# surrealdb/surrealdb

Hardware: AMD Instinct MI355X
Metric: knn_qps (higher is better)
Workload: dtype f32; 1 GPU; brute-force cosine KNN, 10000000 rows/GPU x 768-dim f32, K=10, single query (BASELINE configs[1]); batch=0, rows_total=10000000, rows_per_gpu=10000000, dim=768, k=10, distance=cosine, parallelism=single

## Files before the change

surrealdb_amd/csrc/sdbv.hip:

```cpp

#include <hip/hip_runtime.h>
#include <rocblas/rocblas.h>

#include <algorithm>
#include <atomic>
#include <cfloat>
#include <chrono>
#include <cmath>
#include <cstdint>
#include <deque>
#include <limits>
#include <memory>
#include <thread>
#include <unordered_set>
#include <cstdio>
#include <cstring>
#include <map>
#include <mutex>
#include <queue>
#include <set>
#include <string>
#include <unordered_map>
#include <vector>

// ... 360 lines not shown
	sum.f = __fadd_rn(sum.f, __fadd_rn(p[0].f, p[4].f));                        \
	sum.f = __fadd_rn(sum.f, __fadd_rn(p[1].f, p[5].f));                        \
	sum.f = __fadd_rn(sum.f, __fadd_rn(p[2].f, p[6].f));                        \
	sum.f = __fadd_rn(sum.f, __fadd_rn(p[3].f, p[7].f));
				COMB(x) COMB(y) COMB(z) COMB(w)
#undef COMB
				for (; k8 < d; k8++) {
					const float4 v =
					    *(const float4 *)(cm + (uint64_t)k8 * n_pad + r0);
					const float qk = qs[k8];
					sum.x = __fadd_rn(sum.x, __fmul_rn(v.x, qk));
					sum.y = __fadd_rn(sum.y, __fmul_rn(v.y, qk));
					sum.z = __fadd_rn(sum.z, __fmul_rn(v.z, qk));
					sum.w = __fadd_rn(sum.w, __fmul_rn(v.w, qk));
				}
				const float s[4] = {sum.x, sum.y, sum.z, sum.w};
#pragma unroll
				for (int c = 0; c < ROWS_PER_LANE; c++) {
					double den = q_norm * norms[r0 + c < n_pad ? r0 + c : 0];
					dist[c] = 1.0 - (double)s[c] / den;
				}
			} else {
				float4 acc = make_float4(0.f, 0.f, 0.f, 0.f);
				for (uint32_t kk = 0; kk < d; kk++) {
					const float4 v =
					    *(const float4 *)(cm + (uint64_t)kk * n_pad + r0);
					const float qk = qs[kk];
					float dx = v.x - qk, dy = v.y - qk, dz = v.z - qk,
					      dw = v.w - qk;
					acc.x = __fadd_rn(acc.x, __fmul_rn(dx, dx));
					acc.y = __fadd_rn(acc.y, __fmul_rn(dy, dy));
					acc.z = __fadd_rn(acc.z, __fmul_rn(dz, dz));
					acc.w = __fadd_rn(acc.w, __fmul_rn(dw, dw));
				}
				const float s[4] = {acc.x, acc.y, acc.z, acc.w};
#pragma unroll
				for (int c = 0; c < ROWS_PER_LANE; c++)
					dist[c] = sqrt((double)s[c]);
			}
		}

		uint64_t kk_key = kth_key;
		uint32_t kk_row = kth_row;
		int full = (topk_n >= (int)k);
#pragma unroll
		for (int c = 0; c < ROWS_PER_LANE; c++) {
			if (!valid[c])
				continue;
			uint64_t key = d_total_key(dist[c]);
			uint32_t row32 = (uint32_t)(r0 + c);
			bool take = !full || key < kk_key || (key == kk_key && row32 < kk_row);
			if (take) {
				int idx = atomicAdd(&cnt, 1);
				buf[idx].key = key;
				buf[idx].dist = dist[c];
				buf[idx].row = row32;
			}
		}
		__syncthreads();

		if (cnt > 0) {
			int m = cnt;
			for (int i = threadIdx.x; i < topk_n; i += THREADS)
				buf[m + i] = topk[i];
			int total = m + topk_n;
			__syncthreads();
			int new_n;
			block_select_topk(buf, total, topk, (int)k, &new_n);
			if (threadIdx.x == 0) {
				topk_n = new_n;
				if (new_n >= (int)k) {
					kth_key = topk[k - 1].key;
					kth_row = topk[k - 1].row;
				}
				cnt = 0;
			}
		}
		__syncthreads();
	}

	scan_topk_write(topk, topk_n, k, ids, block_out);
}

__device__ __forceinline__ static void merge_slice(
    Cand *__restrict__ block_out, uint64_t total, uint32_t k,
    uint64_t per_block, Cand *__restrict__ out) {
	__shared__ uint64_t red_key[THREADS / 64];
	__shared__ uint64_t red_id[THREADS / 64];
	__shared__ long red_idx[THREADS / 64];
	const int lane = threadIdx.x & 63;
	const int wave = threadIdx.x >> 6;
	const uint64_t s0 = (uint64_t)blockIdx.x * per_block;
	const uint64_t s1 = s0 + per_block < total ? s0 + per_block : total;
	out += (uint64_t)blockIdx.x * k;
	if (s0 >= total) {
		for (uint32_t i = threadIdx.x; i < k; i += THREADS) {
			out[i].dist = __longlong_as_double(0x7FF0000000000000LL);
			out[i].id = ~0ULL;
		}
		return;
	}
	for (int slot = 0; slot < (int)k; slot++) {
		uint64_t bk = ~0ULL;
		uint64_t bid = ~0ULL;
		long bi = -1;
		for (uint64_t i = s0 + threadIdx.x; i < s1; i += THREADS) {
			uint64_t ck = d_total_key(block_out[i].dist);
			uint64_t cid = block_out[i].id;
			if (ck < bk || (ck == bk && cid < bid)) {
				bk = ck;
				bid = cid;
				bi = (long)i;
			}
		}
		for (int off = 32; off > 0; off >>= 1) {
			uint64_t ok = __shfl_down(bk, off);
			uint64_t oid = __shfl_down(bid, off);
			long oi = __shfl_down(bi, off);
			if (ok < bk || (ok == bk && oid < bid)) {
				bk = ok;
				bid = oid;
				bi = oi;
			}
		}
		if (lane == 0) {
			red_key[wave] = bk;
			red_id[wave] = bid;
			red_idx[wave] = bi;
		}
		__syncthreads();
		if (threadIdx.x == 0) {
			uint64_t bbk = ~0ULL, bbid = ~0ULL;
			long best = -1;
			for (int w = 0; w < THREADS / 64; w++) {
				if (red_idx[w] < 0)
					continue;
				if (red_key[w] < bbk ||
				    (red_key[w] == bbk && red_id[w] < bbid)) {
					bbk = red_key[w];
					bbid = red_id[w];
					best = red_idx[w];
				}
			}
			if (best < 0) {
				out[slot].dist =
				    __longlong_as_double(0x7FF0000000000000LL);
				out[slot].id = ~0ULL;
			} else {
				out[slot] = block_out[best];
				block_out[best].dist =
				    __longlong_as_double(0x7FF0000000000000LL);
				block_out[best].id = ~0ULL;
			}
		}
		__syncthreads();
	}
}

__global__ __launch_bounds__(THREADS) void k_merge(
    Cand *__restrict__ block_out, uint64_t total, uint32_t k,
    uint64_t per_block, Cand *__restrict__ out) {
	merge_slice(block_out, total, k, per_block, out);
}

#define PF_ROWS_PER_LANE 8
#define PF_TILE (THREADS * PF_ROWS_PER_LANE)
#define PF_CAND_CAP 16384u
#define PF_RESCORE_BLOCKS 2048
#define PF_NORM_MIN 0x1p-30
#define PF_NORM_MAX 0x1p30

__host__ __device__ static inline uint32_t pf_bf16_bits(uint32_t u) {
	return (u + 0x7FFFu + ((u >> 16) & 1u)) >> 16;
}

__host__ __device__ static inline float pf_eps(uint32_t d) {
	return 1.01f * (0x1p-8f + 2.0f * (float)(d + 8) * 0x1p-24f) + 0x1p-20f;
}

__device__ static inline uint32_t d_key32(float x) {
	uint32_t b = __float_as_uint(x);
	return (b >> 31) ? ~b : (b | 0x80000000u);
}
__device__ static inline float d_unkey32(uint32_t k) {
	return __uint_as_float((k >> 31) ? (k & 0x7FFFFFFFu) : ~k);
}

__global__ void k_shadow(const float *__restrict__ cm,
                         const double *__restrict__ norms,
                         uint16_t *__restrict__ sh, float *__restrict__ pinv,
                         uint64_t n, uint64_t n_pad, uint64_t sn_pad,
                         uint32_t d) {
	uint64_t r0 = ((uint64_t)blockIdx.x * blockDim.x + threadIdx.x) *
	              PF_ROWS_PER_LANE;
	if (r0 >= sn_pad)
		return;
	const bool in_cm = r0 < n_pad;
	uint32_t bad = 0;
	for (uint32_t k = 0; k < d; k++) {
		float4 a = make_float4(0.f, 0.f, 0.f, 0.f), b = a;
		if (in_cm) {
			a = *(const float4 *)(cm + (uint64_t)k * n_pad + r0);
			b = *(const float4 *)(cm + (uint64_t)k * n_pad + r0 + 4);
		}
		const float v[8] = {a.x, a.y, a.z, a.w, b.x, b.y, b.z, b.w};
		uint32_t h[8];
#pragma unroll
		for (int c = 0; c < 8; c++) {
			uint32_t u = __float_as_uint(v[c]);
			h[c] = pf_bf16_bits(u) & 0xFFFFu;
			if ((u & 0x7F800000u) == 0x7F800000u ||
			    (h[c] & 0x7F80u) == 0x7F80u)
				bad |= 1u << c;
		}
		uint4 o;
		o.x = h[0] | (h[1] << 16);
		o.y = h[2] | (h[3] << 16);
		o.z = h[4] | (h[5] << 16);
		o.w = h[6] | (h[7] << 16);
		*(uint4 *)(sh + (uint64_t)k * sn_pad + r0) = o;
	}
#pragma unroll
	for (int c = 0; c < 8; c++) {
		uint64_t r = r0 + c;
		float inv = __uint_as_float(0x7FC00000u);
		if (r < n && !((bad >> c) & 1u)) {
			double nm = norms[r];
			if (nm >= PF_NORM_MIN && nm <= PF_NORM_MAX)
				inv = (float)(1.0 / nm);
		}
		pinv[r] = inv;
	}
}

__device__ static void pf_block_select(uint64_t *buf, int total,
                                       uint64_t *topk, int k, int *out_n) {
	__shared__ uint64_t red_v[THREADS / 64];
	__shared__ int red_i[THREADS / 64];
	const int lane = threadIdx.x & 63;
	const int wave = threadIdx.x >> 6;
	int out = total < k ? total : k;
	for (int slot = 0; slot < out; slot++) {
		uint64_t bv = ~0ULL;
// ... 880 lines not shown
		}
	} else {
		if (threadIdx.x == 0) {
			float acc = 0.f;
			for (uint32_t kk = 0; kk < d; kk++) {
				float diff = xs[kk] - qs[kk];
				acc = __fadd_rn(acc, __fmul_rn(diff, diff));
			}
			Cand o;
			o.dist = sqrt((double)acc);
			o.id = ids[r];
			*out = o;
		}
	}
}

template <int METRIC>
__device__ __forceinline__ static void rows_exact(
    const float *__restrict__ cm, const double *__restrict__ norms,
    const uint64_t *__restrict__ ids, uint64_t n_pad, uint32_t d,
    const float *__restrict__ qg, double q_norm,
    const uint32_t *__restrict__ rows, uint32_t cnt, Cand *__restrict__ out,
    float *qs, float *xs, float *ps) {
	for (uint32_t i = threadIdx.x; i < d; i += 64)
		qs[i] = qg[i];
	for (uint32_t c = blockIdx.x; c < cnt; c += gridDim.x)
		rows_exact_one<METRIC>(cm, norms, ids, n_pad, d, q_norm, rows[c],
		                       out + c, qs, xs, ps);
}

template <int METRIC>
__global__ __launch_bounds__(64) void k_pf_rescore(
    const float *__restrict__ cm, const double *__restrict__ norms,
    const uint64_t *__restrict__ ids, uint64_t n_pad, uint32_t d,
    const float *__restrict__ qg, double q_norm,
    const uint32_t *__restrict__ cand_cnt,
    const uint32_t *__restrict__ cand_rows, Cand *__restrict__ out) {
	__shared__ float qs[MAX_D];
	__shared__ float xs[MAX_D];
	__shared__ float ps[8];
	const uint32_t cnt = *cand_cnt;
	if (cnt > PF_CAND_CAP || blockIdx.x >= cnt)
		return;
	rows_exact<METRIC>(cm, norms, ids, n_pad, d, qg, q_norm, cand_rows, cnt,
	                   out, qs, xs, ps);
}

template <int METRIC>
__global__ __launch_bounds__(64) void k_rows_exact(
    const float *__restrict__ cm, const double *__restrict__ norms,
    const uint64_t *__restrict__ ids, uint64_t n_pad, uint32_t d,
    const float *__restrict__ qg, double q_norm,
    const uint32_t *__restrict__ rows, uint32_t cnt, Cand *__restrict__ out) {
	__shared__ float qs[MAX_D];
	__shared__ float xs[MAX_D];
	__shared__ float ps[8];
	rows_exact<METRIC>(cm, norms, ids, n_pad, d, qg, q_norm, rows, cnt, out,
	                   qs, xs, ps);
}

__global__ __launch_bounds__(THREADS) void k_pf_final(
    Cand *__restrict__ cands, const uint32_t *__restrict__ cand_cnt,
    uint32_t k, Cand *__restrict__ out) {
	const uint32_t raw = *cand_cnt;
	const uint64_t total = raw > PF_CAND_CAP ? 0 : raw;
	if (threadIdx.x == 0) {
		out[k].dist = 0.0;
		out[k].id = raw;
	}
	merge_slice(cands, total, k, total, out);
}

#define PF4_LIST_CAP 262144u
#define PF4_BLOCK_LIST 8192
#define PF4_PASSES 4
#ifndef PF4_REFINE_LANES
#define PF4_REFINE_LANES 32
#endif

__global__ __launch_bounds__(64) void k_pf4_threshold(
    const float *__restrict__ cm, const double *__restrict__ norms,
    const uint64_t *__restrict__ ids, uint64_t n_pad, uint32_t d,
    const float *__restrict__ qg, double q_norm,
    const Cand *__restrict__ approx_top, Cand *__restrict__ out) {
	__shared__ float qs[MAX_D];
	__shared__ float xs[MAX_D];
	__shared__ float ps[8];
	const uint64_t r = approx_top[blockIdx.x].id;
	if (r == ~0ULL) {
		if (threadIdx.x == 0) {
			Cand o;
			o.dist = __longlong_as_double(0x7FF0000000000000LL);
			o.id = ~0ULL;
			out[blockIdx.x] = o;
		}
		return;
	}
	for (uint32_t i = threadIdx.x; i < d; i += 64)
		qs[i] = qg[i];
	rows_exact_one<0>(cm, norms, ids, n_pad, d, q_norm, (uint32_t)r,
	                  out + blockIdx.x, qs, xs, ps);
}

__device__ __forceinline__ static double pf4_threshold(
    const Cand *__restrict__ thr, uint32_t k, unsigned long long *key) {
	if (threadIdx.x == 0)
		*key = 0;
	__syncthreads();
	if (threadIdx.x < k)
		atomicMax(key, (unsigned long long)d_total_key(thr[threadIdx.x].dist));
	__syncthreads();
	const uint64_t kb = *key;
	return __longlong_as_double(
	    (long long)((kb >> 63) ? (kb & 0x7FFFFFFFFFFFFFFFULL) : ~kb));
}

__global__ __launch_bounds__(THREADS) void k_pf4_compact(
    const float *__restrict__ scores, uint64_t n,
    const Cand *__restrict__ thr, uint32_t k, uint32_t list_cap,
    uint32_t *__restrict__ list_cnt, uint32_t *__restrict__ list_rows) {
	__shared__ uint32_t rows[PF4_BLOCK_LIST];
	__shared__ uint32_t cnt, base;
	__shared__ unsigned long long tkey;
	if (threadIdx.x == 0)
		cnt = 0;
	const double T = pf4_threshold(thr, k, &tkey);
	const uint64_t ngrp = (n + 3) / 4;
	const uint64_t round = (uint64_t)THREADS * PF4_PASSES;
	for (uint64_t g0 = (uint64_t)blockIdx.x * round;;
	     g0 += (uint64_t)gridDim.x * round) {
		const bool last = g0 >= ngrp;
		float4 s[PF4_PASSES];
#pragma unroll
		for (int p = 0; p < PF4_PASSES; p++) {
			const uint64_t g = g0 + (uint64_t)p * THREADS + threadIdx.x;
			if (g < ngrp)
				s[p] = *(const float4 *)(scores + g * 4);
		}
#pragma unroll
		for (int p = 0; p < PF4_PASSES; p++) {
			const uint64_t g = g0 + (uint64_t)p * THREADS + threadIdx.x;
			if (g >= ngrp)
				continue;
			const float v[4] = {s[p].x, s[p].y, s[p].z, s[p].w};
#pragma unroll
			for (int c = 0; c < 4; c++) {
				const uint64_t r = g * 4 + c;
				if (r < n && !((double)v[c] > T))
					rows[atomicAdd(&cnt, 1u)] = (uint32_t)r;
			}
		}
		__syncthreads();
		const uint32_t m = cnt;
		__syncthreads();
		if (m > PF4_BLOCK_LIST - 4 * THREADS * PF4_PASSES || (last && m > 0)) {
			if (threadIdx.x == 0) {
				base = atomicAdd(list_cnt, m);
				cnt = 0;
			}
			__syncthreads();
			for (uint32_t i = threadIdx.x; i < m; i += THREADS)
				if (base + i < list_cap)
					list_rows[base + i] = rows[i];
			__syncthreads();
		}
		if (last)
			break;
	}
}

__global__ __launch_bounds__(THREADS) void k_pf4_refine(
// ... 1946 lines not shown
		return SDBV_ERR_NO_TABLE;
	it->second.order = order;
	return SDBV_OK;
}

static int ensure_query_scratch(sdbv_ctx *ctx, uint32_t d, uint64_t nblocks,
                                uint32_t k) {
	if (ctx->q_cap < d) {
		if (ctx->q_dev)
			(void)hipFree(ctx->q_dev);
		const size_t qb = d * sizeof(float) +
		                  (size_t)((d + 31) / 32) * PF6_QWORDS * sizeof(uint32_t);
		HIP_CHECK(ctx, hipMalloc(&ctx->q_dev, qb));
		if (ctx->q_pin)
			(void)hipHostFree(ctx->q_pin);
		HIP_CHECK(ctx, hipHostMalloc(&ctx->q_pin, qb));
		ctx->q_cap = d;
	}
	uint64_t need = nblocks * k * sizeof(Cand);
	if (ctx->block_out_cap < need) {
		if (ctx->block_out)
			(void)hipFree(ctx->block_out);
		HIP_CHECK(ctx, hipMalloc(&ctx->block_out, need));
		ctx->block_out_cap = need;
	}
	if (!ctx->final_out)
		HIP_CHECK(ctx, hipMalloc(&ctx->final_out, MAX_K * sizeof(Cand)));
	if (!ctx->merge_tmp)
		HIP_CHECK(ctx,
		          hipMalloc(&ctx->merge_tmp, 32 * MAX_K * sizeof(Cand)));
	return SDBV_OK;
}

static int stage_query(sdbv_ctx *ctx, const float *q, uint32_t d,
                       size_t q_bytes) {
	std::memcpy(ctx->q_pin, q, d * sizeof(float));
	HIP_CHECK(ctx, hipMemcpyAsync(ctx->q_dev, ctx->q_pin, q_bytes,
	                              hipMemcpyHostToDevice, ctx->stream));
	return SDBV_OK;
}

static void copy_results(const Cand *host_out, uint32_t m, uint64_t *out_ids,
                         double *out_dists, uint32_t *out_n) {
	*out_n = m;
	for (uint32_t i = 0; i < m; i++) {
		out_ids[i] = host_out[i].id;
		out_dists[i] = host_out[i].dist;
	}
}

static uint64_t scan_grid(uint64_t n, uint64_t *rows_per_block) {
	uint64_t tiles = (n + TILE - 1) / TILE;
	uint64_t nblocks = tiles < 2048 ? tiles : 2048;
	if (nblocks == 0)
		nblocks = 1;
	uint64_t tiles_per_block = (tiles + nblocks - 1) / nblocks;
	*rows_per_block = tiles_per_block * TILE;
	return (n + *rows_per_block - 1) / *rows_per_block;
}

static void launch_scan(sdbv_ctx *ctx, Table &t, uint32_t k, double q_norm,
                        uint64_t nblocks, uint64_t rows_per_block,
                        const uint64_t *mask) {
#define LAUNCH_SCAN(M, MASKED)                                                 \
	hipLaunchKernelGGL((k_scan<M, MASKED>), dim3((uint32_t)nblocks),           \
	                   dim3(THREADS), 0, ctx->stream, t.cm, t.norms, t.n,      \
	                   t.n_pad, t.d, ctx->q_dev, q_norm, k, rows_per_block,    \
	                   (Cand *)ctx->block_out, t.ids_dev, mask)
	const bool cosine = t.metric == SDBV_METRIC_COSINE;
	if (mask) {
		if (cosine)
			LAUNCH_SCAN(0, true);
		else
			LAUNCH_SCAN(1, true);
	} else {
		if (cosine)
			LAUNCH_SCAN(0, false);
		else
			LAUNCH_SCAN(1, false);
	}
#undef LAUNCH_SCAN
}

static void launch_merge_tree(sdbv_ctx *ctx, uint64_t nblocks, uint32_t k) {
	uint64_t total = nblocks * k;
	const uint64_t G = 32;
	if (total > 4096 && nblocks > G) {
		uint64_t per = ((nblocks + G - 1) / G) * k;
		hipLaunchKernelGGL(k_merge, dim3((uint32_t)G), dim3(THREADS), 0,
		                   ctx->stream, (Cand *)ctx->block_out, total, k, per,
		                   (Cand *)ctx->merge_tmp);
		hipLaunchKernelGGL(k_merge, dim3(1), dim3(THREADS), 0, ctx->stream,
		                   (Cand *)ctx->merge_tmp, G * k, k, G * k,
		                   (Cand *)ctx->final_out);
	} else {
		hipLaunchKernelGGL(k_merge, dim3(1), dim3(THREADS), 0, ctx->stream,
		                   (Cand *)ctx->block_out, total, k, total,
		                   (Cand *)ctx->final_out);
	}
}

static void launch_all_dists(sdbv_ctx *ctx, Table &t, const float *q,
                             double *dout) {
	uint64_t nb = (t.n + THREADS - 1) / THREADS;
	double q_norm = t.metric == SDBV_METRIC_COSINE
	                    ? sqrt((double)h_sumsq_f32(q, t.d))
	                    : 0;
	double q_mean = t.metric == SDBV_METRIC_PEARSON ? h_mean_f32(q, t.d) : 0;
#define LAUNCH_AD(M)                                                       \
	hipLaunchKernelGGL(k_all_dists<M>, dim3((uint32_t)nb), dim3(THREADS), \
	                   0, ctx->stream, t.cm, t.norms, t.n, t.n_pad, t.d,  \
	                   ctx->q_dev, q_norm, t.order, q_mean, dout)
	switch (t.metric) {
	case SDBV_METRIC_COSINE: LAUNCH_AD(0); break;
	case SDBV_METRIC_EUCLIDEAN: LAUNCH_AD(1); break;
	case SDBV_METRIC_MANHATTAN: LAUNCH_AD(2); break;
	case SDBV_METRIC_CHEBYSHEV: LAUNCH_AD(3); break;
	case SDBV_METRIC_HAMMING: LAUNCH_AD(4); break;
	case SDBV_METRIC_JACCARD:
		hipLaunchKernelGGL(k_jaccard_dists, dim3((uint32_t)t.n), dim3(256),
		                   0, ctx->stream, t.cm, t.n, t.n_pad, t.d,
		                   ctx->q_dev, dout);
		break;
	case SDBV_METRIC_MINKOWSKI: LAUNCH_AD(6); break;
	case SDBV_METRIC_PEARSON: LAUNCH_AD(7); break;
	}
#undef LAUNCH_AD
}

static int knn_large_k(sdbv_ctx *ctx, Table &t, const float *q, uint32_t d,
                       uint32_t k, const uint64_t *allow, uint64_t *out_ids,
                       double *out_dists, uint32_t *out_n) {
	int rc = ensure_query_scratch(ctx, d, 1, 1);
	if (rc != SDBV_OK)
		return rc;
	rc = stage_query(ctx, q, d, d * sizeof(float));
	if (rc != SDBV_OK)
		return rc;
	double *dout = nullptr;
	HIP_CHECK(ctx, hipMalloc(&dout, t.n * sizeof(double)));
	HIP_CHECK(ctx, hipEventRecord(ctx->ev0, ctx->stream));
	launch_all_dists(ctx, t, q, dout);
	HIP_CHECK(ctx, hipEventRecord(ctx->ev1, ctx->stream));
	std::vector<double> hd(t.n);
	std::vector<uint64_t> hids(t.n);
	if (hipMemcpyAsync(hd.data(), dout, t.n * sizeof(double),
	                   hipMemcpyDeviceToHost, ctx->stream) != hipSuccess ||
	    hipMemcpyAsync(hids.data(), t.ids_dev, t.n * sizeof(uint64_t),
	                   hipMemcpyDeviceToHost, ctx->stream) != hipSuccess ||
	    hipStreamSynchronize(ctx->stream) != hipSuccess ||
	    hipGetLastError() != hipSuccess) {
		(void)hipFree(dout);
		ctx->err = "knn_large_k: device error";
		return SDBV_ERR_HIP;
	}
	(void)hipFree(dout);
	float ms = 0;
	(void)hipEventElapsedTime(&ms, ctx->ev0, ctx->ev1);
	ctx->stats.last_scan_kernel_ms = ms;
	ctx->stats.last_merge_kernel_ms = 0;
	if (!allow)
		ctx->stats.last_rows_scanned = t.n;
	auto tkey = [](double x) {
		uint64_t bits;
		std::memcpy(&bits, &x, 8);
		return (bits >> 63) ? ~bits : (bits | 0x8000000000000000ULL);
	};
	std::priority_queue<std::pair<uint64_t, uint64_t>> heap;
	for (uint64_t r = 0; r < t.n; r++) {
		if (allow && !((allow[r >> 6] >> (r & 63)) & 1ULL))
			continue;
		std::pair<uint64_t, uint64_t> e{tkey(hd[r]), r};
		if (heap.size() < k) {
			heap.push(e);
// ... 301 lines not shown
			nb = 2048;
		if (nb == 0)
			nb = 1;
		hipLaunchKernelGGL(k_pf_compact, dim3((uint32_t)nb), dim3(THREADS), 0,
		                   ctx->stream, ctx->pf_scores, t.n,
		                   (const Cand *)ctx->final_out, k,
		                   kind == 1 ? pf_eps(t.d) : 0.0f, cand_cnt,
		                   ctx->pf_rows);
		if (kind == 5)
			hipLaunchKernelGGL(k_pf_rescore<1>, dim3(PF_RESCORE_BLOCKS),
			                   dim3(64), 0, ctx->stream, t.cm, t.norms,
			                   t.ids_dev, t.n_pad, t.d, ctx->q_dev, q_norm,
			                   cand_cnt, ctx->pf_rows, (Cand *)ctx->pf_cands);
		else
			hipLaunchKernelGGL(k_pf_rescore<0>, dim3(PF_RESCORE_BLOCKS),
			                   dim3(64), 0, ctx->stream, t.cm, t.norms,
			                   t.ids_dev, t.n_pad, t.d, ctx->q_dev, q_norm,
			                   cand_cnt, ctx->pf_rows, (Cand *)ctx->pf_cands);
	}
	HIP_CHECK(ctx, hipEventRecord(ctx->ev3, ctx->stream));
	hipLaunchKernelGGL(k_pf_final, dim3(1), dim3(THREADS), 0, ctx->stream,
	                   (Cand *)ctx->pf_cands, cand_cnt, k, res);
	HIP_CHECK(ctx, hipEventRecord(ctx->ev4, ctx->stream));
	HIP_CHECK(ctx, hipMemcpyAsync(host_out, res, (k + 1) * sizeof(Cand),
	                              hipMemcpyDeviceToHost, ctx->stream));
	HIP_CHECK(ctx, hipStreamSynchronize(ctx->stream));
	HIP_CHECK(ctx, hipGetLastError());
	*ncand = (uint32_t)host_out[k].id;

	float ms_pre = 0, ms_sel = 0, ms_rescore = 0, ms_final = 0;
	(void)hipEventElapsedTime(&ms_pre, ctx->ev0, ctx->ev1);
	(void)hipEventElapsedTime(&ms_sel, ctx->ev1, ctx->ev2);
	(void)hipEventElapsedTime(&ms_rescore, ctx->ev2, ctx->ev3);
	(void)hipEventElapsedTime(&ms_final, ctx->ev3, ctx->ev4);
	ctx->stats.last_scan_kernel_ms = (double)ms_pre + ms_rescore;
	ctx->stats.last_merge_kernel_ms = (double)ms_sel + ms_final;
	if (!mask)
		ctx->stats.last_rows_scanned = t.n;
	return SDBV_OK;
}

static uint32_t pf4_list_max() {
	uint64_t cap = PF4_LIST_CAP;
	const char *e = getenv("SDBV_SCAN_PREFILTER_H4_LIST_MAX");
	if (e && *e) {
		uint64_t v = strtoull(e, nullptr, 10);
		if (v < cap)
			cap = v;
	}
	return (uint32_t)cap;
}

static int knn_prefilter_h4(sdbv_ctx *ctx, Table &t, uint32_t k, double q_norm,
                            const PfQ6 &q6, uint32_t list_cap, Cand *host_out,
                            uint32_t *ncand, uint32_t *nstage1) {
	const Shadow &sh = t.sh;
	int rc = ensure_prefilter_scratch(ctx, sh.sn_pad);
	if (rc != SDBV_OK)
		return rc;
	if (!ctx->pf4_list)
		HIP_CHECK(ctx, hipMalloc(&ctx->pf4_list,
		                         PF4_LIST_CAP * sizeof(uint32_t)));
	if (!ctx->pf4_thr)
		HIP_CHECK(ctx, hipMalloc(&ctx->pf4_thr, MAX_K * sizeof(Cand)));

	uint64_t rows_per_block = 0;
	const uint64_t nblocks =
	    prefilter_grid(ctx, t.n, 4, false, &rows_per_block);
	Cand *res = (Cand *)ctx->pf_res;
	uint32_t *cand_cnt = (uint32_t *)&res[MAX_K + 1];
	const uint32_t ngroups = (t.d + 31) / 32;
	const uint32_t *qd = (const uint32_t *)(ctx->q_dev + t.d);
	const Cand *thr = (const Cand *)ctx->pf4_thr;

	HIP_CHECK(ctx, hipEventRecord(ctx->ev0, ctx->stream));
	hipLaunchKernelGGL((k_prefilter_i6<false, true>), dim3((uint32_t)nblocks),
	                   dim3(THREADS), 0, ctx->stream,
	                   (const uint4 *)sh.plane_h(), (const uint2 *)nullptr,
	                   sh.pscale(), sh.peps4(), sh.xsum_h(), t.n, sh.sn_pad,
	                   ngroups, qd, q6.qscale, q6.qeps, q6.bias4, k,
	                   rows_per_block, ctx->pf_scores, (Cand *)ctx->block_out,
	                   cand_cnt, (const uint64_t *)nullptr);
	HIP_CHECK(ctx, hipEventRecord(ctx->ev1, ctx->stream));
	launch_merge_tree(ctx, nblocks, k);
	HIP_CHECK(ctx, hipEventRecord(ctx->ev2, ctx->stream));
	{
		hipLaunchKernelGGL(k_pf4_threshold, dim3(k), dim3(64), 0, ctx->stream,
		                   t.cm, t.norms, t.ids_dev, t.n_pad, t.d, ctx->q_dev,
		                   q_norm, (const Cand *)ctx->final_out,
		                   (Cand *)ctx->pf4_thr);
		uint64_t ngrp = (t.n + 3) / 4;
		uint64_t nb = (ngrp + THREADS * PF4_PASSES - 1) / (THREADS * PF4_PASSES);
		if (nb > 512)
			nb = 512;
		if (nb == 0)
			nb = 1;
		hipLaunchKernelGGL(k_pf4_compact, dim3((uint32_t)nb), dim3(THREADS), 0,
		                   ctx->stream, ctx->pf_scores, t.n, thr, k, list_cap,
		                   cand_cnt + 1, ctx->pf4_list);
		hipLaunchKernelGGL(k_pf4_refine, dim3(2048), dim3(THREADS), 0,
		                   ctx->stream, (const uint4 *)sh.plane_h(),
		                   (const uint2 *)sh.plane_l(t.d), sh.pscale(),
		                   sh.peps(), sh.xsum(), sh.sn_pad, ngroups, qd,
		                   q6.qscale, q6.qeps, q6.bias, thr, k, list_cap,
		                   cand_cnt + 1, ctx->pf4_list, cand_cnt,
		                   ctx->pf_rows);
		hipLaunchKernelGGL(k_pf_rescore<0>, dim3(PF_RESCORE_BLOCKS), dim3(64),
		                   0, ctx->stream, t.cm, t.norms, t.ids_dev, t.n_pad,
		                   t.d, ctx->q_dev, q_norm, cand_cnt, ctx->pf_rows,
		                   (Cand *)ctx->pf_cands);
	}
	HIP_CHECK(ctx, hipEventRecord(ctx->ev3, ctx->stream));
	hipLaunchKernelGGL(k_pf_final, dim3(1), dim3(THREADS), 0, ctx->stream,
	                   (Cand *)ctx->pf_cands, cand_cnt, k, res);
	HIP_CHECK(ctx, hipEventRecord(ctx->ev4, ctx->stream));
	HIP_CHECK(ctx, hipMemcpyAsync(host_out, res, (MAX_K + 2) * sizeof(Cand),
	                              hipMemcpyDeviceToHost, ctx->stream));
	HIP_CHECK(ctx, hipStreamSynchronize(ctx->stream));
	HIP_CHECK(ctx, hipGetLastError());
	*ncand = (uint32_t)host_out[k].id;
	uint32_t counters[2];
	std::memcpy(counters, &host_out[MAX_K + 1], sizeof(counters));
	*nstage1 = counters[1];

	float ms_pre = 0, ms_sel = 0, ms_rescore = 0, ms_final = 0;
	(void)hipEventElapsedTime(&ms_pre, ctx->ev0, ctx->ev1);
	(void)hipEventElapsedTime(&ms_sel, ctx->ev1, ctx->ev2);
	(void)hipEventElapsedTime(&ms_rescore, ctx->ev2, ctx->ev3);
	(void)hipEventElapsedTime(&ms_final, ctx->ev3, ctx->ev4);
	ctx->stats.last_scan_kernel_ms = (double)ms_pre + ms_rescore;
	ctx->stats.last_merge_kernel_ms = (double)ms_sel + ms_final;
	ctx->stats.last_rows_scanned = t.n;
	return SDBV_OK;
}

static int knn_exact_scan(sdbv_ctx *ctx, Table &t, uint32_t k, double q_norm,
                          uint64_t nblocks, uint64_t rows_per_block,
                          Cand *host_out) {
	HIP_CHECK(ctx, hipEventRecord(ctx->ev0, ctx->stream));
	launch_scan(ctx, t, k, q_norm, nblocks, rows_per_block, nullptr);
	HIP_CHECK(ctx, hipEventRecord(ctx->ev1, ctx->stream));
	launch_merge_tree(ctx, nblocks, k);
	HIP_CHECK(ctx, hipEventRecord(ctx->ev2, ctx->stream));
	HIP_CHECK(ctx, hipMemcpyAsync(host_out, ctx->final_out, k * sizeof(Cand),
	                              hipMemcpyDeviceToHost, ctx->stream));
	HIP_CHECK(ctx, hipStreamSynchronize(ctx->stream));
	HIP_CHECK(ctx, hipGetLastError());

	float ms_scan = 0, ms_merge = 0;
	(void)hipEventElapsedTime(&ms_scan, ctx->ev0, ctx->ev1);
	(void)hipEventElapsedTime(&ms_merge, ctx->ev1, ctx->ev2);
	ctx->stats.last_scan_kernel_ms = ms_scan;
	ctx->stats.last_merge_kernel_ms = ms_merge;
	ctx->stats.last_rows_scanned = t.n;
	return SDBV_OK;
}

int sdbv_knn_bruteforce(sdbv_ctx *ctx, uint64_t table, const float *q,
                        uint32_t d, uint32_t k, uint64_t *out_ids,
                        double *out_dists, uint32_t *out_n) {
	std::lock_guard<std::mutex> lk(ctx->mu);
	auto it = ctx->tables.find(table);
	if (it == ctx->tables.end())
		return SDBV_ERR_NO_TABLE;
	Table &t = it->second;
	if (d != t.d)
		return SDBV_ERR_BAD_ARG;
	if (k == 0 || k > (1u << 22))
		return SDBV_ERR_BAD_ARG;
	ctx->stats.last_scan_path = 0;
	ctx->stats.last_prefilter_candidates = 0;
	ctx->stats.last_prefilter_stage1 = 0;
	if (k > MAX_K || t.metric > SDBV_METRIC_EUCLIDEAN)
// ... 4728 lines not shown
```

Baseline: 1181 queries/s.

## Replace iterative argmin merge with radix-select top-k and fold final merge into threshold

Swaps the k-pass block argmin merge, which rescans the whole slice once per output slot, for a byte-wise radix select over (key,id). The select uses shared-memory histograms and prefix sums to find the k-th element, then does a small rank sort. The second single-block merge launch is removed: each threshold block now redoes the final top-k selection over the 32*k partial results itself. This cuts per-slot passes and one kernel launch, at the cost of extra shared memory, more complex code, and k blocks each repeating the same small selection.

```diff
diff --git a/surrealdb_amd/csrc/sdbv.hip b/surrealdb_amd/csrc/sdbv.hip
--- a/surrealdb_amd/csrc/sdbv.hip
+++ b/surrealdb_amd/csrc/sdbv.hip
@@ -466,14 +466,228 @@
 	scan_topk_write(topk, topk_n, k, ids, block_out);
 }
 
+struct SliceSel {
+	uint32_t hist[256];
+	uint32_t wsum[4];
+	unsigned long long k_and, k_or;
+	uint64_t pk, pid;
+	uint32_t need;
+	uint32_t state;
+	uint32_t pend;
+	uint32_t nsel, neq;
+	uint64_t skey[MAX_K], sid[MAX_K];
+};
+
+__device__ __forceinline__ static bool slice_under(uint64_t key, uint64_t id,
+                                                   uint64_t pk, uint64_t pid,
+                                                   uint32_t p) {
+	if (p == 0)
+		return true;
+	if (p < 8)
+		return (key >> (64 - 8 * p)) == (pk >> (64 - 8 * p));
+	if (key != pk)
+		return false;
+	if (p == 8)
+		return true;
+	return (id >> (128 - 8 * p)) == (pid >> (128 - 8 * p));
+}
+
+__device__ __forceinline__ static bool slice_below(uint64_t key, uint64_t id,
+                                                   uint64_t pk, uint64_t pid,
+                                                   uint32_t p) {
+	if (p <= 8)
+		return p == 8 ? key < pk : (key >> (64 - 8 * p)) < (pk >> (64 - 8 * p));
+	if (key != pk)
+		return key < pk;
+	return p == 16 ? id < pid
+	               : (id >> (128 - 8 * p)) < (pid >> (128 - 8 * p));
+}
+
+template <int NT, int E>
+__device__ __forceinline__ static void block_select_slice(
+    const Cand *__restrict__ in, uint64_t len, uint32_t k, Cand *out,
+    SliceSel *S) {
+	static_assert(NT >= MAX_K && NT <= 256 && 256 % NT == 0 && E < 32, "");
+	constexpr int BPT = 256 / NT;
+	const uint32_t tid = threadIdx.x;
+	const uint32_t lane = tid & 63, wave = tid >> 6;
+	uint64_t ek[E + 1], eid[E + 1];
+	uint32_t vm = 0;
+
+	for (uint64_t c0 = 0; c0 == 0 || c0 < len; c0 += (uint64_t)NT * E) {
+		vm &= 1u << E;
+#pragma unroll
+		for (int e = 0; e < E; e++) {
+			const uint64_t i = c0 + (uint64_t)e * NT + tid;
+			ek[e] = ~0ULL;
+			eid[e] = ~0ULL;
+			if (i < len) {
+				const Cand c = in[i];
+				ek[e] = d_total_key(c.dist);
+				eid[e] = c.id;
+				if (ek[e] != ~0ULL || eid[e] != ~0ULL)
+					vm |= 1u << e;
+			}
+		}
+		uint64_t ka = ~0ULL, ko = 0;
+#pragma unroll
+		for (int e = 0; e <= E; e++)
+			if ((vm >> e) & 1u) {
+				ka &= ek[e];
+				ko |= ek[e];
+			}
+		for (int off = 32; off > 0; off >>= 1) {
+			ka &= __shfl_xor(ka, off);
+			ko |= __shfl_xor(ko, off);
+		}
+		if (tid == 0) {
+			S->k_and = ~0ULL;
+			S->k_or = 0;
+			S->nsel = 0;
+			S->neq = 0;
+			S->state = 0;
+		}
+#pragma unroll
+		for (int b = 0; b < BPT; b++)
+			S->hist[tid * BPT + b] = 0;
+		__syncthreads();
+		if (lane == 0) {
+			atomicAnd(&S->k_and, (unsigned long long)ka);
+			atomicOr(&S->k_or, (unsigned long long)ko);
+		}
+		__syncthreads();
+		const uint64_t kx = S->k_and ^ S->k_or;
+		uint32_t p = S->k_and > S->k_or ? 0u
+		             : kx == 0         ? 8u
+		                               : (uint32_t)__clzll((long long)kx) / 8u;
+		uint64_t pk = p == 0 ? 0 : S->k_and & (~0ULL << (64 - 8 * p));
+		uint64_t pid = 0;
+		uint32_t need = k;
+		uint32_t state = 0;
+
+		for (; p < 16; p++) {
+			const uint32_t sh = p < 8 ? 56 - 8 * p : 120 - 8 * p;
+#pragma unroll
+			for (int e = 0; e <= E; e++)
+				if (((vm >> e) & 1u) &&
+				    slice_under(ek[e], eid[e], pk, pid, p))
+					atomicAdd(&S->hist[((p < 8 ? ek[e] : eid[e]) >> sh) & 255u],
+					          1u);
+			__syncthreads();
+			uint32_t c[BPT], mine = 0;
+#pragma unroll
+			for (int b = 0; b < BPT; b++) {
+				c[b] = S->hist[tid * BPT + b];
+				S->hist[tid * BPT + b] = 0;
+				mine += c[b];
+			}
+			uint32_t incl = mine;
+			for (int off = 1; off < 64; off <<= 1) {
+				const uint32_t o = __shfl_up(incl, off);
+				if (lane >= (uint32_t)off)
+					incl += o;
+			}
+			if (lane == 63)
+				S->wsum[wave] = incl;
+			__syncthreads();
+			uint32_t acc = incl - mine, total = 0;
+#pragma unroll
+			for (int w = 0; w < NT / 64; w++) {
+				const uint32_t ws = S->wsum[w];
+				acc += (uint32_t)w < wave ? ws : 0u;
+				total += ws;
+			}
+			if (total < need) {
+				if (tid == 0)
+					S->state = 2;
+			} else {
+#pragma unroll
+				for (int b = 0; b < BPT; b++) {
+					if (c[b] != 0 && acc < need && acc + c[b] >= need) {
+						const uint64_t dg = (uint64_t)(tid * BPT + b) << sh;
+						S->pk = p < 8 ? pk | dg : pk;
+						S->pid = p < 8 ? 0 : pid | dg;
+						S->need = need - acc;
+						S->pend = p + 1;
+						S->state = (c[b] == need - acc || p == 15) ? 1u : 0u;
+					}
+					acc += c[b];
+				}
+			}
+			__syncthreads();
+			state = S->state;
+			if (state == 2)
+				break;
+			pk = S->pk;
+			pid = S->pid;
+			need = S->need;
+			if (state == 1)
+				break;
+		}
+		const uint32_t pend = state == 1 ? S->pend : 0;
+#pragma unroll
+		for (int e = 0; e <= E; e++) {
+			if (!((vm >> e) & 1u))
+				continue;
+			bool take = state == 2;
+			if (!take) {
+				take = slice_below(ek[e], eid[e], pk, pid, pend);
+				if (!take && slice_under(ek[e], eid[e], pk, pid, pend))
+					take = atomicAdd(&S->neq, 1u) < need;
+			}
+			if (take) {
+				const uint32_t pos = atomicAdd(&S->nsel, 1u);
+				if (pos < MAX_K) {
+					S->skey[pos] = ek[e];
+					S->sid[pos] = eid[e];
+				}
+			}
+		}
+		__syncthreads();
+		const uint32_t m = S->nsel;
+		if (c0 + (uint64_t)NT * E < len) {
+			vm = 0;
+			if (tid < m) {
+				ek[E] = S->skey[tid];
+				eid[E] = S->sid[tid];
+				vm = 1u << E;
+			}
+			__syncthreads();
+			continue;
+		}
+		if (tid < m) {
+			const uint64_t kt = S->skey[tid], it = S->sid[tid];
+			uint32_t rank = 0;
+			for (uint32_t j = 0; j < m; j++) {
+				const uint64_t kj = S->skey[j], ij = S->sid[j];
+				rank += (kj < kt ||
+				         (kj == kt && (ij < it || (ij == it && j < tid))))
+				            ? 1u
+				            : 0u;
+			}
+			Cand o;
+			o.dist = __longlong_as_double(
+			    (long long)((kt >> 63) ? (kt & 0x7FFFFFFFFFFFFFFFULL) : ~kt));
+			o.id = it;
+			if (rank > 0 && kt > 0xFFF0000000000000ULL) {
+				o.dist = __longlong_as_double(0x7FF0000000000000LL);
+				o.id = ~0ULL;
+			}
+			out[rank] = o;
+		} else if (tid < k) {
+			Cand o;
+			o.dist = __longlong_as_double(0x7FF0000000000000LL);
+			o.id = ~0ULL;
+			out[tid] = o;
+		}
+		__syncthreads();
+	}
+}
+
 __device__ __forceinline__ static void merge_slice(
-    Cand *__restrict__ block_out, uint64_t total, uint32_t k,
+    const Cand *__restrict__ block_out, uint64_t total, uint32_t k,
     uint64_t per_block, Cand *__restrict__ out) {
-	__shared__ uint64_t red_key[THREADS / 64];
-	__shared__ uint64_t red_id[THREADS / 64];
-	__shared__ long red_idx[THREADS / 64];
-	const int lane = threadIdx.x & 63;
-	const int wave = threadIdx.x >> 6;
+	__shared__ SliceSel sel;
 	const uint64_t s0 = (uint64_t)blockIdx.x * per_block;
 	const uint64_t s1 = s0 + per_block < total ? s0 + per_block : total;
 	out += (uint64_t)blockIdx.x * k;
@@ -484,65 +698,11 @@
 		}
 		return;
 	}
-	for (int slot = 0; slot < (int)k; slot++) {
-		uint64_t bk = ~0ULL;
-		uint64_t bid = ~0ULL;
-		long bi = -1;
-		for (uint64_t i = s0 + threadIdx.x; i < s1; i += THREADS) {
-			uint64_t ck = d_total_key(block_out[i].dist);
-			uint64_t cid = block_out[i].id;
-			if (ck < bk || (ck == bk && cid < bid)) {
-				bk = ck;
-				bid = cid;
-				bi = (long)i;
-			}
-		}
-		for (int off = 32; off > 0; off >>= 1) {
-			uint64_t ok = __shfl_down(bk, off);
-			uint64_t oid = __shfl_down(bid, off);
-			long oi = __shfl_down(bi, off);
-			if (ok < bk || (ok == bk && oid < bid)) {
-				bk = ok;
-				bid = oid;
-				bi = oi;
-			}
-		}
-		if (lane == 0) {
-			red_key[wave] = bk;
-			red_id[wave] = bid;
-			red_idx[wave] = bi;
-		}
-		__syncthreads();
-		if (threadIdx.x == 0) {
-			uint64_t bbk = ~0ULL, bbid = ~0ULL;
-			long best = -1;
-			for (int w = 0; w < THREADS / 64; w++) {
-				if (red_idx[w] < 0)
-					continue;
-				if (red_key[w] < bbk ||
-				    (red_key[w] == bbk && red_id[w] < bbid)) {
-					bbk = red_key[w];
-					bbid = red_id[w];
-					best = red_idx[w];
-				}
-			}
-			if (best < 0) {
-				out[slot].dist =
-				    __longlong_as_double(0x7FF0000000000000LL);
-				out[slot].id = ~0ULL;
-			} else {
-				out[slot] = block_out[best];
-				block_out[best].dist =
-				    __longlong_as_double(0x7FF0000000000000LL);
-				block_out[best].id = ~0ULL;
-			}
-		}
-		__syncthreads();
-	}
+	block_select_slice<THREADS, 16>(block_out + s0, s1 - s0, k, out, &sel);
 }
 
 __global__ __launch_bounds__(THREADS) void k_merge(
-    Cand *__restrict__ block_out, uint64_t total, uint32_t k,
+    const Cand *__restrict__ block_out, uint64_t total, uint32_t k,
     uint64_t per_block, Cand *__restrict__ out) {
 	merge_slice(block_out, total, k, per_block, out);
 }
@@ -1589,11 +1749,20 @@
     const float *__restrict__ cm, const double *__restrict__ norms,
     const uint64_t *__restrict__ ids, uint64_t n_pad, uint32_t d,
     const float *__restrict__ qg, double q_norm,
-    const Cand *__restrict__ approx_top, Cand *__restrict__ out) {
+    const Cand *__restrict__ approx_top, uint32_t fold_total, uint32_t k,
+    Cand *__restrict__ out) {
 	__shared__ float qs[MAX_D];
 	__shared__ float xs[MAX_D];
 	__shared__ float ps[8];
-	const uint64_t r = approx_top[blockIdx.x].id;
+	__shared__ SliceSel sel;
+	__shared__ Cand top[MAX_K];
+	uint64_t r;
+	if (fold_total > 0) {
+		block_select_slice<64, 16>(approx_top, fold_total, k, top, &sel);
+		r = top[blockIdx.x].id;
+	} else {
+		r = approx_top[blockIdx.x].id;
+	}
 	if (r == ~0ULL) {
 		if (threadIdx.x == 0) {
 			Cand o;
@@ -3706,14 +3875,21 @@
 #undef LAUNCH_SCAN
 }
 
-static void launch_merge_tree(sdbv_ctx *ctx, uint64_t nblocks, uint32_t k) {
+static void launch_merge_tree(sdbv_ctx *ctx, uint64_t nblocks, uint32_t k,
+                              uint32_t *fold = nullptr) {
 	uint64_t total = nblocks * k;
 	const uint64_t G = 32;
+	if (fold)
+		*fold = 0;
 	if (total > 4096 && nblocks > G) {
 		uint64_t per = ((nblocks + G - 1) / G) * k;
 		hipLaunchKernelGGL(k_merge, dim3((uint32_t)G), dim3(THREADS), 0,
 		                   ctx->stream, (Cand *)ctx->block_out, total, k, per,
 		                   (Cand *)ctx->merge_tmp);
+		if (fold) {
+			*fold = (uint32_t)(G * k);
+			return;
+		}
 		hipLaunchKernelGGL(k_merge, dim3(1), dim3(THREADS), 0, ctx->stream,
 		                   (Cand *)ctx->merge_tmp, G * k, k, G * k,
 		                   (Cand *)ctx->final_out);
@@ -4181,13 +4357,15 @@
 	                   rows_per_block, ctx->pf_scores, (Cand *)ctx->block_out,
 	                   cand_cnt, (const uint64_t *)nullptr);
 	HIP_CHECK(ctx, hipEventRecord(ctx->ev1, ctx->stream));
-	launch_merge_tree(ctx, nblocks, k);
+	uint32_t fold = 0;
+	launch_merge_tree(ctx, nblocks, k, &fold);
 	HIP_CHECK(ctx, hipEventRecord(ctx->ev2, ctx->stream));
 	{
 		hipLaunchKernelGGL(k_pf4_threshold, dim3(k), dim3(64), 0, ctx->stream,
 		                   t.cm, t.norms, t.ids_dev, t.n_pad, t.d, ctx->q_dev,
-		                   q_norm, (const Cand *)ctx->final_out,
-		                   (Cand *)ctx->pf4_thr);
+		                   q_norm,
+		                   (const Cand *)(fold ? ctx->merge_tmp : ctx->final_out),
+		                   fold, k, (Cand *)ctx->pf4_thr);
 		uint64_t ngrp = (t.n + 3) / 4;
 		uint64_t nb = (ngrp + THREADS * PF4_PASSES - 1) / (THREADS * PF4_PASSES);
 		if (nb > 512)
```

Measured after the change: 1221 queries/s (median of 6 runs). 3.5% higher.
